# mp3guy/Kintinuous

Hardware: NVIDIA H100
Metric: frames/s 640x480 into 512^3 TSDF (ICP-only tracker) (higher is better)
Workload: dtype f32

## Files before the change

### kintinuous_b200/csrc/kt_capi.cu

```cuda
#include "kt_ops.h"
#include "kt_solve.cuh"
#include "kt_pgo.hpp"
#include "../../include/kintinuous_b200.h"
#include <cstring>
#include <cstddef>
#include <mutex>
#include <vector>
#include <algorithm>

using namespace kt;

namespace {

Intr intr4(const float* k) { Intr r = {k[0], k[1], k[2], k[3]}; return r; }
Mat33 mat33(const float* m) { Mat33 r; r.r0 = make_float3(m[0], m[1], m[2]); r.r1 = make_float3(m[3], m[4], m[5]); r.r2 = make_float3(m[6], m[7], m[8]); return r; }
cudaStream_t st(void* s) { return (cudaStream_t)s; }

struct OpScratch { Allocations mem; OdomState* state; float* partials; int* ipartials; unsigned int* counter; OdomState* host_state;
                   DeviceBuffer<float> ztable; SliceWorkspace slice_ws; MeshWorkspace mesh_ws; DeviceBuffer<unsigned long long> mesh_cells; SurfWorkspace surf_ws; PnpWorkspace pnp_ws;
                   SliceWorkspace fit_ws; DeviceBuffer<int> place_ints; };
enum { KT_MAX_DEVICES = 64 };
OpScratch* g_ops_dev[KT_MAX_DEVICES];
std::mutex g_ops_mu;
OpScratch& ops_scratch()
{
    int dev = 0;
    if (cudaGetDevice(&dev) != cudaSuccess || dev < 0 || dev >= KT_MAX_DEVICES) dev = 0;
    if (!g_ops_dev[dev]) g_ops_dev[dev] = new OpScratch();
    return *g_ops_dev[dev];
}
#define g_ops (ops_scratch())
#define KT_OPS_LOCK() std::lock_guard<std::mutex> _ops_lock(g_ops_mu)

int ensure_scratch()
{
    if (g_ops.host_state) return 0;
    Allocations m; const char* W = "operator scratch";
    OdomState* state; float* partials; int* ipartials; unsigned int* counter; OdomState* host_state;
    int r;
    if ((r = m.device(&state, 1, W)) || (r = m.device(&partials, (size_t)MAX_PARTIALS * 32, W)) || (r = m.device(&ipartials, (size_t)MAX_PARTIALS * 2, W)) ||
        (r = m.device(&counter, 1, W)) || (r = m.pinned(&host_state, 1, W))) return r;
    KT_CUDA(cudaMemset(state, 0, sizeof(OdomState)));
    OpScratch& o = g_ops;
    o.mem = std::move(m); o.state = state; o.partials = partials; o.ipartials = ipartials; o.counter = counter; o.host_state = host_state;
    return 0;
}
int check_vol(const char* who, int vol)
{
    if (vol <= 0 || vol % 8 != 0) { set_error("%s: vol %d is not a positive multiple of 8", who, vol); return KT_ERR_INVALID; }
    return KT_OK;
}

int ensure_ztable(int vol)
{
    const size_t n = vol > 0 ? (size_t)2 * vol : 0;
    return g_ops.ztable.grow(n, n, "operator z table");
}

}

extern "C" {

int kt_op_bilateral(const uint16_t* src, uint16_t* dst, int rows, int cols, void* s)
{ int r = bilateral(src, dst, rows, cols, st(s)); if (r) return r; KT_CUDA(cudaStreamSynchronize(st(s))); return KT_OK; }

int kt_op_pyrdown(const uint16_t* src, uint16_t* dst, int sr, int sc, void* s)
{ int r = pyrdown(src, dst, sr, sc, st(s)); if (r) return r; KT_CUDA(cudaStreamSynchronize(st(s))); return KT_OK; }

int kt_op_create_vmap(const float* k, const uint16_t* depth, float* vmap, int rows, int cols, void* s)
{ int r = create_vmap(intr4(k), depth, vmap, rows, cols, st(s)); if (r) return r; KT_CUDA(cudaStreamSynchronize(st(s))); return KT_OK; }

int kt_op_create_nmap(const float* vmap, float* nmap, int rows, int cols, void* s)
{ int r = create_nmap(vmap, nmap, rows, cols, st(s)); if (r) return r; KT_CUDA(cudaStreamSynchronize(st(s))); return KT_OK; }

int kt_op_create_maps(const float* k, const uint16_t* depth, float* vmap, float* nmap, int rows, int cols, void* s)
{
    MapsLevel L; L.depth = depth; L.vmap = vmap; L.nmap = nmap; L.rows = rows; L.cols = cols; L.k = intr4(k); L.vstale = 0; L.nstale = 0;
    int r = create_maps_pyramid(&L, 1, st(s)); if (r) return r;
    KT_CUDA(cudaStreamSynchronize(st(s))); return KT_OK;
}

int kt_op_frontend(const uint16_t* depth_raw, const uint8_t* rgb, int rows, int cols, const float* k, int angle_color,
                   uint16_t* const* depths4, float* const* vmaps4, float* const* nmaps4, float* depth_scaled, float* cw, float* rgbf,
                   float* const* depth_m4, uint8_t* const* intensity4, int16_t* const* dIdx4, int16_t* const* dIdy4, void* s)
{
    if (!depth_raw || !rgb || !depths4 || !vmaps4 || !nmaps4) { set_error("kt_op_frontend: null argument"); return KT_ERR_INVALID; }
    int r = bilateral_scale(depth_raw, depths4[0], depth_scaled, rows, cols, intr4(k), angle_color != 0, st(s)); if (r) return r;
    FrontendArgs fa;
    fa.depth_f = depths4[0]; fa.depth_raw = depth_raw; fa.rgb = rgb; fa.rows = rows; fa.cols = cols; fa.k = intr4(k);
    fa.depths = depths4; fa.vmaps = vmaps4; fa.nmaps = nmaps4; fa.vstale = 0; fa.nstale = 0;
    fa.cw = cw; fa.rgbf = (float4*)rgbf; fa.angle_color = angle_color != 0; fa.cut_off = 6000;
// ... 8 lines not shown

int kt_op_resize_vmap(const float* in, float* out, int in_rows, int in_cols, void* s)
{ int r = resize_map(in, out, in_rows, in_cols, false, st(s)); if (r) return r; KT_CUDA(cudaStreamSynchronize(st(s))); return KT_OK; }

int kt_op_resize_nmap(const float* in, float* out, int in_rows, int in_cols, void* s)
{ int r = resize_map(in, out, in_rows, in_cols, true, st(s)); if (r) return r; KT_CUDA(cudaStreamSynchronize(st(s))); return KT_OK; }

int kt_op_icp_step(const float* Rcurr, const float* tcurr, const float* vmap_curr, const float* nmap_curr,
                   const float* Rprev_inv, const float* tprev, const float* k,
                   const float* vmap_g_prev, const float* nmap_g_prev, int rows, int cols,
                   float dist_thres, float angle_thres, float* A_host, float* b_host, float* residual_host, void* s)
{
    KT_OPS_LOCK();
    int r = ensure_scratch(); if (r) return r;
    OdomState* h = g_ops.host_state;
    std::memset(h, 0, sizeof(OdomState));
    std::memcpy(h->Rcurr, Rcurr, 36); std::memcpy(h->tcurr, tcurr, 12); std::memcpy(h->Rprev_inv, Rprev_inv, 36); std::memcpy(h->tprev, tprev, 12);
    KT_CUDA(cudaMemcpyAsync(g_ops.state, h, sizeof(OdomState), cudaMemcpyHostToDevice, st(s)));
    IcpLevelArgs a = {vmap_curr, nmap_curr, vmap_g_prev, nmap_g_prev, rows, cols, intr4(k), dist_thres, angle_thres};
    r = icp_iteration(a, g_ops.state, g_ops.partials, 0, 0, st(s)); if (r) return r;
    KT_CUDA(cudaMemcpyAsync(h->sums_icp, (char*)g_ops.state + offsetof(OdomState, sums_icp), 32 * sizeof(float), cudaMemcpyDeviceToHost, st(s)));
    KT_CUDA(cudaStreamSynchronize(st(s)));
    unpack_normal_equations(h->sums_icp, A_host, b_host);
    residual_host[0] = h->sums_icp[27]; residual_host[1] = h->sums_icp[28];
    return KT_OK;
}

int kt_op_integrate(const uint16_t* depth_raw, int rows, int cols, const float* k, const float* vs,
                    const float* Rinv, const float* t, float trunc, int16_t* tsdf, uint8_t* color, int vol,
                    const int* wrap, const uint8_t* rgb, const float* nmap_curr, int angle_color, float* depth_scaled, void* s)
{
    int r = check_vol("kt_op_integrate", vol); if (r) return r;
    KT_OPS_LOCK();
    r = ensure_ztable(vol); if (r) return r;
    r = scale_depth(depth_raw, depth_scaled, rows, cols, intr4(k), angle_color != 0, st(s)); if (r) return r;
    IntegrateArgs a; a.cw = 0; a.rgbf = 0; a.reset_words = 0; a.reset_count = 0; a.reset_stride = 1;
    a.depth_scaled = depth_scaled; a.rows = rows; a.cols = cols; a.k = intr4(k); a.volume_size = make_float3(vs[0], vs[1], vs[2]);
    a.Rinv = mat33(Rinv); a.t = make_float3(t[0], t[1], t[2]); a.trunc = trunc; a.tsdf = tsdf; a.color = color; a.vol = vol;
    a.wrap = make_int3(wrap[0], wrap[1], wrap[2]); a.rgb = rgb; a.nmap_curr = nmap_curr; a.angle_color = angle_color != 0;
    a.multi = 0; a.vv = single_volume(tsdf, color, vol);
    r = integrate(a, g_ops.ztable.get(), st(s)); if (r) return r;
    KT_CUDA(cudaStreamSynchronize(st(s)));
    return KT_OK;
}

int kt_op_raycast(const float* k, const float* R, const float* t, float trunc, const float* vs,
                  const int16_t* tsdf, int vol, float* vmap, float* nmap, int rows, int cols,
                  const int* wrap, uint8_t* vmap_color, const uint8_t* color, void* s)
{
    if (vol > 0) { if (int r = check_cell_size(make_float3(vs[0], vs[1], vs[2]), vol)) return r; }
    if (int r = check_vol("kt_op_raycast", vol)) return r;
    RaycastArgs a = {};
    a.k = intr4(k); a.R = mat33(R); a.t = make_float3(t[0], t[1], t[2]); a.trunc = trunc; a.volume_size = make_float3(vs[0], vs[1], vs[2]);
    a.tsdf = tsdf; a.color = color; a.vol = vol; a.wrap = make_int3(wrap[0], wrap[1], wrap[2]);
    for (int l = 0; l < LEVELS; ++l) { a.vmap[l] = vmap; a.nmap[l] = nmap; }
    a.rows = rows; a.cols = cols; a.vmap_color = vmap_color; a.n_levels = 1;
    int r = raycast(a, st(s)); if (r) return r;
    KT_CUDA(cudaStreamSynchronize(st(s)));
    return KT_OK;
}

int kt_op_extract_slice(const int16_t* tsdf, const float* vs, int vol, kt_point_xyzrgb* out, size_t capacity,
                        const int* wrap, const uint8_t* color, int minX, int maxX, int minY, int maxY, int minZ, int maxZ,
                        int subsample, const int* real_wrap, size_t* count, void* s)
{
    int r = check_vol("kt_op_extract_slice", vol); if (r) return r;
    KT_OPS_LOCK();
    r = ensure_scratch(); if (r) return r;
    KT_CUDA(cudaMemsetAsync(g_ops.counter, 0, sizeof(unsigned int), st(s)));
    r = extract_slice(tsdf, make_float3(vs[0], vs[1], vs[2]), vol, out, capacity, make_int3(wrap[0], wrap[1], wrap[2]), color,
                      minX, maxX, minY, maxY, minZ, maxZ, subsample, make_int3(real_wrap[0], real_wrap[1], real_wrap[2]), g_ops.counter, st(s));
    if (r) return r;
    unsigned int n = 0;
    KT_CUDA(cudaMemcpyAsync(&n, g_ops.counter, sizeof(n), cudaMemcpyDeviceToHost, st(s)));
// ... 296 lines not shown
```

### kintinuous_b200/csrc/kt_ops.h

```cpp
#pragma once
#include "kt_common.cuh"
#include "kt_mem.hpp"
#include <functional>

struct kt_deform_report;
struct kt_pgo_report;
struct kt_weld_report;
struct kt_global_mesh_report;

namespace kt {

static const int LEVELS = 4;
static const int MAX_GPUS = 8;

struct VolumeView {
    int16_t* tsdf[MAX_GPUS];
    uint8_t* color[MAX_GPUS];
    int world, rank, bshift, nshift;
};
__host__ __device__ __forceinline__ int vv_owner(const VolumeView& v, int sz) { return (sz >> v.bshift) & (v.world - 1); }
__host__ __device__ __forceinline__ int vv_local_plane(const VolumeView& v, int sz)
{ return ((sz >> (v.bshift + v.nshift)) << v.bshift) | (sz & ((1 << v.bshift) - 1)); }
inline VolumeView single_volume(int16_t* tsdf, uint8_t* color, int V)
{
// ... 61 lines not shown

int icp_frame(const IcpLevelArgs* levels, const int* iters, const float* pose12_host, OdomState* state, unsigned long long* xwords_dev,
              float* trace, int* timeout_dev, long long* prof_dev, float* host_pose, unsigned int host_seq, cudaStream_t s,
              unsigned long long* const* peer_words = 0, int world = 1, int rank = 0);
size_t odom_exchange_words();
int odom_exchange_used(int* stride);
int odom_exchange_reset(unsigned long long* xwords_dev, cudaStream_t s);

struct RgbLevelArgs {
    const int16_t* dIdx; const int16_t* dIdy; const float* last_depth; const float* next_depth;
    const uint8_t* last_image; const uint8_t* next_image; void* corres; const float* cloud;
    int rows, cols; float min_scale, max_depth_delta, fx, fy, sobel_scale; double Kfx, Kfy, Kcx, Kcy;
};
int rgb_residual(const RgbLevelArgs& a, OdomState* state, int* partials, int use_state_warp, cudaStream_t s);
int rgbd_frame(const IcpLevelArgs* icp_levels, const RgbLevelArgs* rgb_levels, const int* iters, int with_icp, const float* pose12_host, OdomState* state,
               unsigned long long* xwords_dev, float* trace, int* timeout_dev, float* host_pose, unsigned int host_seq, cudaStream_t s);
int rgb_iteration(const RgbLevelArgs& a, OdomState* state, float* partials, float* trace, int mode, float sigma_override, cudaStream_t s);
int odom_begin_frame(OdomState* state, const float* pose12_dev, cudaStream_t s);
int reduce_grid_for(int n_items);

int init_volume(int16_t* tsdf, uint8_t* color, int vol, cudaStream_t s);
int init_shared(const VolumeView& vv, int vol, cudaStream_t s);
int clear_volume(int axis, int back, int16_t* tsdf, uint8_t* color, int vol, int current_wrap, int delta_wrap, cudaStream_t s);
int clear_volume_shared(int axis, int back, const VolumeView& vv, int vol, int current_wrap, int delta_wrap, cudaStream_t s);
void clear_range(int axis, int back, int vol, int current_wrap, int delta_wrap, int* first, int* planes);
int scale_depth(const uint16_t* depth, float* scaled, int rows, int cols, const Intr& k, bool angle_color, cudaStream_t s);
struct IntegrateArgs {
    const float* depth_scaled; int rows, cols; Intr k; float3 volume_size; Mat33 Rinv; float3 t; float trunc;
    int16_t* tsdf; uint8_t* color; int vol; int3 wrap; const uint8_t* rgb; const float* nmap_curr; bool angle_color;
    int multi; VolumeView vv;
    float* cw; float4* rgbf;
    unsigned long long* reset_words; int reset_count, reset_stride;
};
int integrate(const IntegrateArgs& a, float* ztable_dev , cudaStream_t s);
struct RaycastArgs {
    Intr k; Mat33 R; float3 t; float trunc; float3 volume_size; const int16_t* tsdf; const uint8_t* color; int vol; int3 wrap;
    float* vmap[LEVELS]; float* nmap[LEVELS]; int rows, cols; uint8_t* vmap_color; int n_levels;
    int multi; VolumeView vv; int tile_row_begin, tile_row_end;
    float* peer_vmap[MAX_GPUS][LEVELS]; float* peer_nmap[MAX_GPUS][LEVELS]; uint8_t* peer_vcol[MAX_GPUS];
};
int raycast(const RaycastArgs& a, cudaStream_t s);
int check_cell_size(const float3& volume_size, int vol);
int extract_slice(const int16_t* tsdf, const float3& volume_size, int vol, void* out, size_t capacity, const int3& wrap,
                  const uint8_t* color, int minX, int maxX, int minY, int maxY, int minZ, int maxZ, int subsample,
                  const int3& real_wrap, unsigned int* counter_dev, cudaStream_t s);
int extract_slice_mg(const VolumeView& vv, const float3& volume_size, int vol, void* out, size_t capacity, const int3& wrap,
                     int minX, int maxX, int minY, int maxY, int minZ, int maxZ, int subsample,
                     const int3& real_wrap, unsigned int* counter_dev, cudaStream_t s);
struct SliceWorkspace {
    DeviceBuffer<unsigned int> mask, word_off, block_tot;
    DeviceBuffer<unsigned char> acc;
    Allocations fixed; unsigned int* bounds = nullptr; unsigned int* bounds_host = nullptr;
};
int process_slice(const void* points_dev , size_t n, int weight_cull, float leaf, int k_search, void* out_dev ,
                  size_t capacity, size_t* count, SliceWorkspace* ws, cudaStream_t s);
struct MeshArgs {
    const int16_t* tsdf; const uint8_t* color; int vol; float3 volume_size; int3 wrap; int3 real_wrap;
    int minX, maxX, minY, maxY, minZ, maxZ; int weight_cull;
};
struct MeshWorkspace {
    DeviceBuffer<unsigned long long> counts;
    DeviceBuffer<unsigned char> tmp;
    DeviceBuffer<unsigned long long> keys;
    Allocations fixed; unsigned long long* totals_host = nullptr;
};
int mesh_count(const MeshArgs& a, MeshWorkspace* ws, size_t* n_verts, size_t* n_tris, cudaStream_t s);
int mesh_emit(const MeshArgs& a, MeshWorkspace* ws, size_t n_verts, void* verts, uint32_t* tris, cudaStream_t s, unsigned long long* vkeys = nullptr,
// ... 71 lines not shown
```

### kintinuous_b200/csrc/kt_tracker.cu

```cuda
#include "kt_ops.h"
#include "kt_shift.hpp"
#include "kt_posegraph.hpp"
#include "kt_deform.hpp"
#include "kt_pgo.hpp"
#include "kt_place.hpp"
#include <cstdlib>
#include "../../include/kintinuous_b200.h"
#include <memory>
#include <vector>
#include <unordered_map>
#include <cstring>
#include <cmath>
#include <climits>
#include <algorithm>
#include <cstdarg>
#include <cstdio>

namespace kt {

static thread_local char g_err[512] = "";
std::atomic<long long> g_launches(0);
void set_error(const char* fmt, ...)
{
    va_list ap; va_start(ap, fmt); vsnprintf(g_err, sizeof(g_err), fmt, ap); va_end(ap);
// ... 114 lines not shown
    int* best; float* d1; float* d2; unsigned char* pass; int* seg_passes;
    float* pn; float* po; float* uv; double* pose; unsigned char* inl; int* ninl; PnpWorkspace pnp_ws;
    MapPyramid maps[2];
    OdomState* state; unsigned long long* xwords; float* trace;
    kt_point_xyzrgb* cloud[2]; kt_point_xyzrgbnormal* cent[2]; double* d2fit; SliceWorkspace ws[2];
    std::vector<std::vector<float> > in_new, in_old;
    ~PlaceStore() { if (stream) cudaStreamSynchronize(stream); }
};

}

using namespace kt;

struct kt_ctx {
    kt_config cfg;
    cudaStream_t stream;
    float size, voxel, trunc;
    float volumeBasis[3], currentGlobalCamera[3];
    int voxelWrap[3];
    int global_time; uint64_t current_utime;
    int overlap, parked;
    std::vector<M3> rmats; std::vector<V3> tvecs;
    std::vector<SliceRec> slices;
    std::vector<kt_dense_pose> dense_poses;
    FILE* pose_log;
    int iterations[LEVELS];
    int16_t* tsdf; uint8_t* color;
    FrameInputs in, in_spare; FrontEnd fe, fe_spare;
    const void* pf_depth; const void* pf_rgb; bool pf_valid;
    bool pf_built;
    bool frontend_ready;
    cudaStream_t stream_copy; cudaEvent_t ev_prefetch, ev_done[2], ev_maps; int last_parity; bool maps_on_stream;
    float* vmaps_g_prev[LEVELS]; float* nmaps_g_prev[LEVELS];
    uint8_t* vmap_curr_color; float* ztable;
    unsigned long long* xwords_dev; bool xwords_clean;
    OdomState* state; float* partials; int* ipartials; float* trace_dev; float* pose12_dev; long long* prof_dev;
    kt_point_xyzrgb* cloud_dev; unsigned int* counter_dev; size_t cloud_capacity; size_t cloud_count;
    PinnedArena slice_arena; cudaStream_t stream_slices; cudaEvent_t ev_cloud_ready, ev_cloud_free; bool cloud_busy;
    int slice_processing, slice_weight_cull; SliceWorkspace slice_ws; DeviceBuffer<kt_point_xyzrgbnormal> proc; size_t proc_count;
    int slice_meshing, mesh_weight_cull; MeshWorkspace mesh_ws; DeviceBuffer<kt_mesh_vertex> mesh_verts; DeviceBuffer<uint32_t> mesh_tris;
    size_t mesh_nv, mesh_nt;
    DeviceBuffer<unsigned long long> mesh_vkeys, mesh_tcells; MeshKeyFrame mesh_frame;
    struct Deformed { kt_point_xyzrgbnormal* processed; kt_mesh_vertex* mesh_verts; };
    std::vector<Deformed> deformed; PinnedArena deform_arena;
    struct Loop { uint64_t time1, time2; double C[16]; std::vector<float> in1, in2; };
    std::vector<Loop> loops; std::vector<kt_dense_pose> pgo_nodes;
    struct MapCorrection { uint64_t time; float tracked[16]; float corrected[16]; };
    MapCorrection map_corr;
    PhotometricPyramid ph_last, ph_next;
    int16_t* nextdIdx[LEVELS]; int16_t* nextdIdy[LEVELS]; float* pointClouds[LEVELS]; void* corresImg[LEVELS];
    float* pose12_host; OdomResult* result_host; float* result_dev_alias; unsigned int pose_seq; float* trace_host; unsigned int* counter_host;
    int trace_iters; int shifted_last;
    bool timing; cudaEvent_t ev[6]; cudaEvent_t ev_icp[2]; cudaEvent_t ev_krn[4]; cudaEvent_t ev_span[2];
    long long launches_at_create;
    Allocations mem;
    int world, rank, local_planes, mg_block;
    uint8_t* arena; size_t arena_bytes;
    size_t off_tsdf, off_color, off_vmap[LEVELS], off_nmap[LEVELS], off_vcol, off_flags, off_xwords;
    bool split_icp;
    uint8_t* peer_arena[MAX_GPUS]; bool connected;
    unsigned int** peer_flags_dev; unsigned int epoch; int* mg_error_dev; int* mg_error_host;
    VolumeView vv;
    float last_int_Rinv[9], last_int_t[3]; int last_int_wrap[3];
    DeviceBuffer<uint8_t> view;
    std::unique_ptr<PlaceStore> place;
    std::unique_ptr<MapVolume> mapvol;
    bool mapvol_restore = false;
// ... 93 lines not shown
        KT_CUDA(cudaEventRecord(c->ev_cloud_free, c->stream_slices));
        c->cloud_busy = true;
    }
    for (int i = 0; i < 3; ++i) s.camera_t[i] = c->currentGlobalCamera[i];
    for (int i = 0; i < 9; ++i) s.camera_R[i] = c->rmats.back().m[i];
    s.utime = c->current_utime;
    c->slices.push_back(std::move(s));
    return 0;
}

void drop_slices(kt_ctx* c)
{
    if (c->stream_slices) cudaStreamSynchronize(c->stream_slices);
    c->slices.clear();
    c->slice_arena.rewind();
    c->cloud_busy = false;
}

bool builds_icp_maps(const kt_config& cfg) { return cfg.odometry == 0 || cfg.odometry == 2 || cfg.angle_color; }

int do_integrate(kt_ctx* c, const M3& Rinv, const V3& t, const int* wrap)
{
    const int rows = c->cfg.rows, cols = c->cfg.cols;
    Intr k = {c->cfg.fx, c->cfg.fy, c->cfg.cx, c->cfg.cy};
    IntegrateArgs a;
    a.depth_scaled = c->fe.depth_scaled; a.rows = rows; a.cols = cols; a.k = k; a.volume_size = make_float3(c->size, c->size, c->size);
    a.Rinv = to_mat33(Rinv.m); a.t = make_float3(t.v[0], t.v[1], t.v[2]); a.trunc = c->trunc;
    a.tsdf = c->tsdf; a.color = c->color; a.vol = c->cfg.vol; a.wrap = make_int3(wrap[0], wrap[1], wrap[2]);
    a.rgb = c->in.rgb; a.nmap_curr = c->fe.maps.nmaps[0]; a.angle_color = c->cfg.angle_color != 0;
    for (int k = 0; k < 9; ++k) c->last_int_Rinv[k] = Rinv.m[k];
    for (int k = 0; k < 3; ++k) { c->last_int_t[k] = t.v[k]; c->last_int_wrap[k] = wrap[k]; }
    a.reset_words = c->xwords_dev; a.reset_count = odom_exchange_used(&a.reset_stride); c->xwords_clean = true;
    a.multi = c->world > 1 ? 1 : 0; a.vv = c->vv; a.cw = builds_icp_maps(c->cfg) ? c->fe.cw : 0; a.rgbf = a.cw ? (float4*)c->fe.rgbf : 0;
    return integrate(a, c->ztable, c->stream);
}

struct OdomMaps { const float* const* vmaps_curr; const float* const* nmaps_curr; const float* const* vmaps_g_prev; const float* const* nmaps_g_prev; };

void odom_level_args(const kt_ctx* c, const OdomMaps& m, int level, IcpLevelArgs* ia, RgbLevelArgs* ra)
{
    const float distThres = 0.10f, angleThres = sinf(20.f * 3.14159254f / 180.f);
    const Intr K = {c->cfg.fx, c->cfg.fy, c->cfg.cx, c->cfg.cy};
    const int lr = c->cfg.rows >> level, lc = c->cfg.cols >> level;
    const Intr kl = intr_level(K, level);
    const IcpLevelArgs icp = {m.vmaps_curr[level], m.nmaps_curr[level], m.vmaps_g_prev[level], m.nmaps_g_prev[level], lr, lc, kl, distThres, angleThres};
    *ia = icp;
    if (c->cfg.odometry == 0) return;
    const double SOBEL_SCALE = 1.0 / std::pow(2.0, 3);
    const int minimumGradientMagnitudes[4] = {12, 5, 3, 1};
    const int div = 1 << level;
    ra->dIdx = c->nextdIdx[level]; ra->dIdy = c->nextdIdy[level]; ra->last_depth = c->ph_last.depth[level]; ra->next_depth = c->ph_next.depth[level];
    ra->last_image = c->ph_last.image[level]; ra->next_image = c->ph_next.image[level]; ra->corres = c->corresImg[level]; ra->cloud = c->pointClouds[level];
    ra->rows = lr; ra->cols = lc;
    ra->min_scale = (float)(std::pow((double)minimumGradientMagnitudes[level], 2.0) / std::pow(SOBEL_SCALE, 2.0));
    ra->max_depth_delta = 0.07f; ra->fx = kl.fx; ra->fy = kl.fy; ra->sobel_scale = (float)SOBEL_SCALE;
    ra->Kfx = (double)K.fx / div; ra->Kfy = (double)K.fy / div; ra->Kcx = (double)K.cx / div; ra->Kcy = (double)K.cy / div;
}

int run_odometry(kt_ctx* c, const OdomMaps& maps, const M3& Rprev, const V3& tprev, M3* Rcurr, V3* tcurr)
{
    const int mode = c->cfg.odometry;
    int r;
    for (int k = 0; k < 9; ++k) c->pose12_host[k] = Rprev.m[k];
    for (int k = 0; k < 3; ++k) c->pose12_host[9 + k] = tprev.v[k];
    IcpLevelArgs la[LEVELS]; RgbLevelArgs ra[LEVELS];
    for (int level = 0; level < LEVELS; ++level) odom_level_args(c, maps, level, &la[level], &ra[level]);
    int total_iters = 0;
// ... 381 lines not shown
        if (dev(&c->arena, off)) return KT_ERR_CUDA;
        KT_CUDA(cudaMemset(c->arena + c->off_flags, 0, 256));
        c->xwords_dev = (unsigned long long*)(c->arena + c->off_xwords);
        KT_CUDA(cudaMemset(c->xwords_dev, 0, odom_exchange_words() * sizeof(unsigned long long))); c->xwords_clean = true;
        c->split_icp = c->world > 1 && getenv("KT_MG_SPLIT_ICP") != nullptr;
        c->tsdf = (int16_t*)(c->arena + c->off_tsdf); c->color = c->arena + c->off_color;
        for (int g = 0; g < MAX_GPUS; ++g) c->peer_arena[g] = c->arena;
        c->connected = (c->world == 1);
        c->epoch = 0;
        c->vv = single_volume(c->tsdf, c->color, cfg->vol);
        c->vv.world = c->world; c->vv.rank = c->rank;
        c->vv.bshift = 0; { int t = c->mg_block; while (t > 1) { t >>= 1; ++c->vv.bshift; } }
        c->vv.nshift = 0; { int t = c->world; while (t > 1) { t >>= 1; ++c->vv.nshift; } }
        if (dev(&c->peer_flags_dev, (size_t)MAX_GPUS)) return KT_ERR_CUDA;
        if (c->mem.mapped(&c->mg_error_host, 1, W)) return KT_ERR_CUDA; *c->mg_error_host = 0;
        KT_CUDA(cudaHostGetDevicePointer((void**)&c->mg_error_dev, c->mg_error_host, 0));
    }
    if (c->in.alloc(c->mem, P, W) || c->in_spare.alloc(c->mem, P, W) || c->fe.alloc(c->mem, P, W) || c->fe_spare.alloc(c->mem, P, W)) return KT_ERR_CUDA;
    if (cfg->odometry != 0 && (c->ph_last.alloc(c->mem, P, W) || c->ph_next.alloc(c->mem, P, W))) return KT_ERR_CUDA;
    if (c->mem.stream(&c->stream_copy, W)) return KT_ERR_CUDA;
    if (event(&c->ev_prefetch, cudaEventDisableTiming)) return KT_ERR_CUDA;
    for (int i = 0; i < 2; ++i) if (event(&c->ev_done[i], cudaEventDisableTiming)) return KT_ERR_CUDA;
    if (event(&c->ev_maps, cudaEventDisableTiming)) return KT_ERR_CUDA; c->maps_on_stream = false;
    c->last_parity = 0;
    for (int l = 0; l < LEVELS; ++l) {
        size_t Pl = P >> (2 * l);
        c->vmaps_g_prev[l] = (float*)(c->arena + c->off_vmap[l]); c->nmaps_g_prev[l] = (float*)(c->arena + c->off_nmap[l]);
        if (cfg->odometry != 0) {
            if (dev(&c->nextdIdx[l], Pl) || dev(&c->nextdIdy[l], Pl)) return KT_ERR_CUDA;
            if (dev(&c->pointClouds[l], Pl * 3)) return KT_ERR_CUDA;
            uint8_t* ci = 0; if (dev(&ci, Pl * 16)) return KT_ERR_CUDA; c->corresImg[l] = ci;
        }
    }
    c->vmap_curr_color = c->arena + c->off_vcol; if (dev(&c->ztable, (size_t)2 * cfg->vol)) return KT_ERR_CUDA;

    if (dev(&c->state, 1) || dev(&c->partials, (size_t)MAX_PARTIALS * 32)) return KT_ERR_CUDA;
    KT_CUDA(cudaMemset(c->partials, 0, (size_t)MAX_PARTIALS * 32 * sizeof(float)));
    if (dev(&c->prof_dev, 64 * 8) || dev(&c->ipartials, (size_t)MAX_PARTIALS * 2)) return KT_ERR_CUDA;
    if (dev(&c->trace_dev, (size_t)MAX_TRACE_ITERS * TRACE_STRIDE) || dev(&c->pose12_dev, 12)) return KT_ERR_CUDA;
    c->cloud_capacity = (size_t)c->cfg.cloud_capacity;
    if (dev(&c->cloud_dev, c->cloud_capacity) || dev(&c->counter_dev, 1)) return KT_ERR_CUDA;
    c->mesh_weight_cull = 8;
    if (!c->slice_arena.alloc(256)) return KT_ERR_CUDA;
    c->slice_arena.rewind();
    if (c->mem.stream(&c->stream_slices, W)) return KT_ERR_CUDA;
    if (event(&c->ev_cloud_ready, cudaEventDisableTiming)) return KT_ERR_CUDA;
    if (event(&c->ev_cloud_free, cudaEventDisableTiming)) return KT_ERR_CUDA;
    if (c->mem.pinned(&c->pose12_host, 12, W)) return KT_ERR_CUDA;
    if (c->mem.mapped(&c->result_host, 1, W)) return KT_ERR_CUDA;
    std::memset(c->result_host, 0, sizeof(OdomResult));
    { void* dp = 0; KT_CUDA(cudaHostGetDevicePointer(&dp, c->result_host, 0)); c->result_dev_alias = (float*)dp; }
    c->pose_seq = 0;
    if (c->mem.pinned(&c->trace_host, (size_t)MAX_TRACE_ITERS * TRACE_STRIDE, W)) return KT_ERR_CUDA;
    if (c->mem.pinned(&c->counter_host, 1, W)) return KT_ERR_CUDA;
    for (int i = 0; i < 6; ++i) if (event(&c->ev[i], cudaEventDefault)) return KT_ERR_CUDA;
    for (int i = 0; i < 2; ++i) if (event(&c->ev_icp[i], cudaEventDefault)) return KT_ERR_CUDA;
    for (int i = 0; i < 4; ++i) if (event(&c->ev_krn[i], cudaEventDefault)) return KT_ERR_CUDA;
    for (int i = 0; i < 2; ++i) if (event(&c->ev_span[i], cudaEventDefault)) return KT_ERR_CUDA;
    int r = kt_reset(c); if (r) return r;
    *out = owner.release();
    return KT_OK;
}

int kt_destroy(kt_ctx* c)
{
    delete c;
    return KT_OK;
// ... 1364 lines not shown
```

### kintinuous_b200/csrc/kt_tsdf.cu

```cuda
#include "kt_ops.h"
#include "kt_replay.cuh"
#include "kt_frustum.hpp"

namespace kt {

namespace {

__global__ void __launch_bounds__(256) fill_zero_u4(uint4* __restrict__ p, size_t n16)
{
    const uint4 z = make_uint4(0, 0, 0, 0);
    for (size_t i = (size_t)blockIdx.x * blockDim.x + threadIdx.x; i < n16; i += (size_t)gridDim.x * blockDim.x) p[i] = z;
}

__global__ void __launch_bounds__(256)
clear_planes_yz_kernel(int16_t* __restrict__ tsdf, uint8_t* __restrict__ color, int V, int axis, int p0, int count, const VolumeView vv)
{
    const int xg = V / 8;
    const size_t total = (size_t)count * V * xg;
    const uint4 z4 = make_uint4(0, 0, 0, 0);
    for (size_t idx = (size_t)blockIdx.x * blockDim.x + threadIdx.x; idx < total; idx += (size_t)gridDim.x * blockDim.x) {
        int g = (int)(idx % xg);
        size_t r = idx / xg;
        int other = (int)(r % V);
        int i = (int)(r / V);
        int plane = p0 + i; if (plane >= V) plane -= V;
        int sy = axis == 1 ? plane : other;
        int sz = axis == 1 ? other : plane;
        *reinterpret_cast<uint4*>(tsdf + ((size_t)sz * V + sy) * V + (size_t)g * 8) = z4;
        if (vv_owner(vv, sz) != vv.rank) continue;
        size_t base = ((size_t)vv_local_plane(vv, sz) * V + sy) * V + (size_t)g * 8;
        uint4* c = reinterpret_cast<uint4*>(color + base * 4);
        c[0] = z4; c[1] = z4;
    }
}

__global__ void __launch_bounds__(256)
clear_planes_x_kernel(int16_t* __restrict__ tsdf, uchar4* __restrict__ color, int V, int p0, int count, const VolumeView vv)
{
    const size_t total = (size_t)count * V * V;
    for (size_t idx = (size_t)blockIdx.x * blockDim.x + threadIdx.x; idx < total; idx += (size_t)gridDim.x * blockDim.x) {
        int i = (int)(idx % count);
        size_t r = idx / count;
        int sx = p0 + i; if (sx >= V) sx -= V;
        const int sz = (int)(r / V), sy = (int)(r - (size_t)sz * V);
        tsdf[r * V + sx] = 0;
        if (vv_owner(vv, sz) != vv.rank) continue;
        color[((size_t)vv_local_plane(vv, sz) * V + sy) * V + sx] = make_uchar4(0, 0, 0, 0);
    }
}

__global__ void __launch_bounds__(256) ztable_kernel(float* __restrict__ table, int V, float cell_z, float t_z, unsigned long long* __restrict__ reset_words, int reset_count, int reset_stride, int seq)
{
    const int i = blockIdx.x * blockDim.x + threadIdx.x;
    if (blockIdx.x == 0) for (int k = threadIdx.x; k < reset_count; k += blockDim.x) reset_words[(size_t)k * reset_stride] = 0ull;
    if (i >= 2 * V) return;
    const int z = i < V ? i : i - V;
    float v = i < V ? __fmaf_rn(0.5f, cell_z, -t_z) : 0.f;
    if (seq) { for (int k = 0; k < z; ++k) v = __fadd_rn(v, cell_z); }
    else v = replay_add(v, cell_z, z);
    table[i] = v;
}

struct IntegrateParams {
    const float* depth_scaled; int rows, cols; Intr k; float3 cell; Mat33 Rinv; float3 t; float trunc;
    int16_t* tsdf; uchar4* color; int V; int3 wrap; const uint8_t* rgb; const float* nmap; bool angle_color;
    const float* ztable; int zchunk;
    const float* cw; const float4* rgbf;
    int lz_lo, lz_hi;
    int z_far_first;
    VolumeView vv;
    int tile_x0, tiles_x, tile_y0, tiles_y;
    int seq_replay;
};

#define KT_MAX_WEIGHT 128
#define KT_RGB_VIEW_ANGLE_WEIGHT 0.75f

__device__ __forceinline__ unsigned int sat_u8_rn(float x)
{
    unsigned int r;
    asm("cvt.rni.sat.u8.f32 %0, %1;" : "=r"(r) : "f"(x));
    return r;
}

template <typename IdxT, int ZU, int MINB, bool PREP = false, bool MG = false>
__global__ void __launch_bounds__(256, MINB)
integrate_kernel(const IntegrateParams p)
{
    const int V = p.V;
    int bx = p.tile_x0 + (int)blockIdx.x; if (bx >= p.tiles_x) bx -= p.tiles_x;
    int by = p.tile_y0 + (int)blockIdx.y; if (by >= p.tiles_y) by -= p.tiles_y;
    const int sx = bx * 32 + threadIdx.x;
    const int sy = by * 8 + threadIdx.y;
    const int z0 = p.lz_lo + (p.z_far_first ? (int)(gridDim.z - 1 - blockIdx.z) : (int)blockIdx.z) * p.zchunk;
    const int z1 = min(z0 + p.zchunk, p.lz_hi);

    const float3 cell_size = p.cell;
    const Intr intr = p.k;
    const Mat33 Rcurr_inv = p.Rinv;
    const float3 tcurr = p.t;
    const float tranc_dist = p.trunc;
    const int cols = p.cols, rows = p.rows;

    if (sx >= V || sy >= V) return;
    int x = sx - p.wrap.x; if (x < 0) x += V;
    int y = sy - p.wrap.y; if (y < 0) y += V;

    float v_g_x = __fmaf_rn(x + 0.5f, cell_size.x, -tcurr.x);
    float v_g_y = __fmaf_rn(y + 0.5f, cell_size.y, -tcurr.y);
    float v_g_z = __fmaf_rn(0.5f, cell_size.z, -tcurr.z);

    float v_g_part_norm = __fmaf_rn(v_g_x, v_g_x, __fmul_rn(v_g_y, v_g_y));

    float v_x = __fmul_rn(__fmaf_rn(Rcurr_inv.r0.z, v_g_z, __fmaf_rn(Rcurr_inv.r0.x, v_g_x, __fmul_rn(Rcurr_inv.r0.y, v_g_y))), intr.fx);
    float v_y = __fmul_rn(__fmaf_rn(Rcurr_inv.r1.z, v_g_z, __fmaf_rn(Rcurr_inv.r1.x, v_g_x, __fmul_rn(Rcurr_inv.r1.y, v_g_y))), intr.fy);
    float v_z = __fmaf_rn(Rcurr_inv.r2.z, v_g_z, __fmaf_rn(Rcurr_inv.r2.x, v_g_x, __fmul_rn(Rcurr_inv.r2.y, v_g_y)));

    float Rcurr_inv_0_z_scaled = Rcurr_inv.r0.z * cell_size.z * intr.fx;
    float Rcurr_inv_1_z_scaled = Rcurr_inv.r1.z * cell_size.z * intr.fy;
    const float m0z = __fmul_rn(Rcurr_inv.r0.z, cell_size.z), m1z = __fmul_rn(Rcurr_inv.r1.z, cell_size.z);

    float tranc_dist_inv = 1.0f / tranc_dist;

    int zlo = z0, zhi = z1;
    {
        const float dqx = Rcurr_inv_0_z_scaled, dqy = Rcurr_inv_1_z_scaled, dqz = Rcurr_inv.r2.z * cell_size.z;
        {
            const float za = (float)(z0 - 3), zb = (float)(z1 + 3);
// ... 8 lines not shown
        float lo = -1e30f, hi = 1e30f;
        const float ca[5] = { v_z,
                              v_x + (intr.cx + 1.5f) * v_z,
                              -(v_x + (intr.cx - cols - 0.5f) * v_z),
                              v_y + (intr.cy + 1.5f) * v_z,
                              -(v_y + (intr.cy - rows - 0.5f) * v_z) };
        const float cb[5] = { dqz,
                              dqx + (intr.cx + 1.5f) * dqz,
                              -(dqx + (intr.cx - cols - 0.5f) * dqz),
                              dqy + (intr.cy + 1.5f) * dqz,
                              -(dqy + (intr.cy - rows - 0.5f) * dqz) };
#pragma unroll
        for (int c = 0; c < 5; ++c) {
            const float a = ca[c], b = cb[c];
            const float eps = 1e-3f * (fabsf(a) + fabsf(b) * V) + 1e-6f;
            if (fabsf(b) * V <= eps) { if (a < -eps) { lo = 1e30f; hi = -1e30f; } }
            else {
                float zc = -(a + eps) / b;
                if (b > 0) lo = fmaxf(lo, zc); else hi = fminf(hi, zc);
            }
        }
        if (lo > hi) return;
        zlo = max(z0, (int)floorf(fmaxf(lo, -4.f)) - 2);
        zhi = min(z1, (int)ceilf(fminf(hi, (float)V + 4.f)) + 3);
        if (zlo >= zhi) return;
    }

    if (p.seq_replay) {
        for (int z = 0; z < zlo; ++z) { v_x = __fmaf_rn(m0z, intr.fx, v_x); v_y = __fmaf_rn(m1z, intr.fy, v_y); }
    } else {
        v_x = replay_fma(v_x, m0z, intr.fx, zlo);
        v_y = replay_fma(v_y, m1z, intr.fy, zlo);
    }
    const float* __restrict__ zt = p.ztable;
    const float* __restrict__ depthScaled = p.depth_scaled;
    const float* __restrict__ nmap_curr = p.nmap;
    const uchar3* __restrict__ colors = reinterpret_cast<const uchar3*>(p.rgb);
    const IdxT P = (IdxT)rows * cols;
    const IdxT plane = (IdxT)V * V;
    const IdxT col_off = (IdxT)sy * V + sx;

    for (int zb = zlo; zb < zhi; zb += ZU) {
        if (MG) {
            int sz = zb + p.wrap.z; if (sz >= V) sz -= V;
            if (vv_owner(p.vv, sz) != p.vv.rank) {
                const int blk = sz >> p.vv.bshift;
                const int foreign = (p.vv.rank - blk - 1) & (p.vv.world - 1);
                int skip = (((blk + 1) << p.vv.bshift) - sz) + (foreign << p.vv.bshift);
                skip = min(skip, zhi - zb);
                if (skip <= 48) { for (int k = 0; k < skip; ++k) { v_x = __fmaf_rn(m0z, intr.fx, v_x); v_y = __fmaf_rn(m1z, intr.fy, v_y); } }
                else { v_x = replay_fma(v_x, m0z, intr.fx, skip); v_y = replay_fma(v_y, m1z, intr.fy, skip); }
                zb += skip - ZU;
                continue;
            }
        }
        float vgz[ZU], Dp[ZU];
        IdxT pix[ZU], addr[ZU], caddr[ZU];
        bool ok[ZU];
        float nx[ZU], nz[ZU];
        int16_t tprev[ZU]; uchar4 cprev[ZU]; uchar3 rgbv[ZU]; float4 rgbq[ZU];
#pragma unroll
        for (int u = 0; u < ZU; ++u) {
            const int z = zb + u;
            ok[u] = false;
            if (z < zhi) {
                vgz[u] = zt[z];
                const float z_scaled = zt[V + z];
                float inv_z = 1.0f / __fmaf_rn(Rcurr_inv.r2.z, z_scaled, v_z);
                if (!(inv_z < 0)) {
                    int2 coo = { __float2int_rn(__fmaf_rn(v_x, inv_z, intr.cx)), __float2int_rn(__fmaf_rn(v_y, inv_z, intr.cy)) };
                    if (coo.x >= 0 && coo.y >= 0 && coo.x < cols && coo.y < rows) {
                        int sz = z + p.wrap.z; if (sz >= V) sz -= V;
                        ok[u] = true;
                        pix[u] = (IdxT)coo.y * cols + coo.x;
                        addr[u] = (IdxT)sz * plane + col_off;
                        caddr[u] = MG ? (IdxT)vv_local_plane(p.vv, sz) * plane + col_off : addr[u];
                        Dp[u] = depthScaled[pix[u]];
                    }
                }
                v_x = __fmaf_rn(m0z, intr.fx, v_x);
                v_y = __fmaf_rn(m1z, intr.fy, v_y);
            }
        }
        bool upd[ZU], nocol[ZU];
        float tsdf_new[ZU];
#pragma unroll
        for (int u = 0; u < ZU; ++u) {
            upd[u] = false;
            if (ok[u]) {
                float Dp_scaled = Dp[u];
                bool no_color = false;
                if (Dp_scaled < 0.0) { Dp_scaled = -Dp_scaled; no_color = true; }
                float sdf = Dp_scaled - sqrtf(__fmaf_rn(vgz[u], vgz[u], v_g_part_norm));
                if (Dp_scaled != 0 && sdf >= -tranc_dist) {
                    upd[u] = true; nocol[u] = no_color;
                    tsdf_new[u] = fmin(1.0f, sdf * tranc_dist_inv);
                    tprev[u] = p.tsdf[addr[u]];
                    cprev[u] = p.color[caddr[u]];
                    if (PREP) { nx[u] = p.cw[pix[u]]; rgbq[u] = p.rgbf[pix[u]]; }
                    else {
// ... 92 lines not shown
    const int n = delta - current;
    const int an = n < 0 ? -n : n;
    const int base = wrap_base(current, V);
    int p0 = back ? ((base - an) % V + V) % V : base;
    int count = an + 1;
    if (axis == 0) {
        int reach = (an % 16 != 0) ? (an + 16 - an % 16) : an;
        if (count > reach) count = reach;
    }
    if (count > V) count = V;
    *first = p0; *planes = count > 0 ? count : 0;
}

int clear_volume_shared(int axis, int back, const VolumeView& vv, int vol, int current, int delta, cudaStream_t s)
{
    const int V = vol;
    int p0, count;
    clear_range(axis, back, vol, current, delta, &p0, &count);
    if (count <= 0) return 0;
    int16_t* tsdf = vv.tsdf[vv.rank]; uint8_t* color = vv.color[vv.rank];
    if (axis == 0) {
        size_t total = (size_t)count * V * V;
        int grid = (int)((total + 255) / 256 < (size_t)device_info().sm_count * 16 ? (total + 255) / 256 : (size_t)device_info().sm_count * 16);
        clear_planes_x_kernel<<<grid, 256, 0, s>>>(tsdf, (uchar4*)color, V, p0, count, vv);
    } else {
        size_t total = (size_t)count * V * (V / 8);
        int grid = (int)((total + 255) / 256 < (size_t)device_info().sm_count * 16 ? (total + 255) / 256 : (size_t)device_info().sm_count * 16);
        clear_planes_yz_kernel<<<grid, 256, 0, s>>>(tsdf, color, V, axis, p0, count, vv);
    }
    KT_LAUNCH_CHECK();
    return 0;
}

int integrate(const IntegrateArgs& a, float* ztable_dev, cudaStream_t s)
{
    const int V = a.vol;
    float3 cell = make_float3(a.volume_size.x / V, a.volume_size.y / V, a.volume_size.z / V);
    static const bool seq_replay = getenv("KT_INT_SEQ_REPLAY") != nullptr;
    ztable_kernel<<<div_up(2 * V, 256), 256, 0, s>>>(ztable_dev, V, cell.z, a.t.z, a.reset_words, a.reset_words ? a.reset_count : 0, a.reset_stride, seq_replay ? 1 : 0);
    KT_LAUNCH_CHECK();
    IntegrateParams p;
    p.depth_scaled = a.depth_scaled; p.rows = a.rows; p.cols = a.cols; p.k = a.k; p.cell = cell; p.Rinv = a.Rinv; p.t = a.t; p.trunc = a.trunc;
    p.tsdf = a.tsdf; p.color = (uchar4*)a.color; p.V = V; p.wrap = wrap_mod3(a.wrap, V); p.rgb = a.rgb; p.nmap = a.nmap_curr; p.angle_color = a.angle_color;
    static int zu = -1;
    if (zu < 0) { const char* e = getenv("KT_INT_ZU"); zu = e ? atoi(e) : 0; }
    static int prep_knob = -1;
    if (prep_knob < 0) { const char* e = getenv("KT_INT_PREP"); prep_knob = e ? atoi(e) : 1; }
    const bool prep = prep_knob != 0 && a.cw && a.rgbf;
    p.cw = a.cw; p.rgbf = a.rgbf;
    p.ztable = ztable_dev; p.zchunk = V >= 64 ? (V + 15) / 16 : V;
    p.z_far_first = a.Rinv.r2.z > 0.f ? 0 : 1;
    const bool multi = a.multi && a.vv.world > 1;
    p.vv = multi ? a.vv : single_volume(a.tsdf, a.color, V);
    static const bool force64 = getenv("KT_FORCE_IDX64") != nullptr;
    const bool idx32 = !force64 && (size_t)V * V * V <= ((size_t)1 << 31);
    p.lz_lo = 0; p.lz_hi = V;
    p.seq_replay = seq_replay ? 1 : 0;
    p.tiles_x = div_up(V, 32); p.tiles_y = div_up(V, 8); p.tile_x0 = 0; p.tile_y0 = 0;
    dim3 block(32, 8), grid(p.tiles_x, p.tiles_y, div_up(V, p.zchunk));
    static const bool no_box = getenv("KT_INT_NOBOX") != nullptr;
    if (!no_box) {
        const float Rinv9[9] = {a.Rinv.r0.x, a.Rinv.r0.y, a.Rinv.r0.z, a.Rinv.r1.x, a.Rinv.r1.y, a.Rinv.r1.z, a.Rinv.r2.x, a.Rinv.r2.y, a.Rinv.r2.z};
        const float t3[3] = {a.t.x, a.t.y, a.t.z}, k4[4] = {a.k.fx, a.k.fy, a.k.cx, a.k.cy}, cell3[3] = {cell.x, cell.y, cell.z};
        const VoxelBox box = frustum_voxel_box(Rinv9, t3, k4, a.rows, a.cols, V, cell3);
        if (box.empty) return 0;
        p.lz_lo = box.lo[2]; p.lz_hi = box.hi[2] + 1;
        grid.z = div_up(p.lz_hi - p.lz_lo, p.zchunk);
        if (V % 32 == 0) { int n; cyclic_tile_range(box.lo[0], box.hi[0], p.wrap.x, V, 32, &p.tile_x0, &n); grid.x = n; }
        if (V % 8 == 0) { int n; cyclic_tile_range(box.lo[1], box.hi[1], p.wrap.y, V, 8, &p.tile_y0, &n); grid.y = n; }
    }
    if (multi) {
        if (V & (V - 1)) { set_error("integrate: the shared volume needs a power-of-two resolution"); return -1; }
        if (idx32) { if (prep) integrate_kernel<unsigned int, 1, 6, true, true><<<grid, block, 0, s>>>(p); else integrate_kernel<unsigned int, 1, 6, false, true><<<grid, block, 0, s>>>(p); }
        else { if (prep) integrate_kernel<size_t, 1, 6, true, true><<<grid, block, 0, s>>>(p); else integrate_kernel<size_t, 1, 6, false, true><<<grid, block, 0, s>>>(p); }
    } else if (idx32) {
        const int variant = zu ? zu : (V >= 1024 ? 1 : 2);
        if (prep && (variant == 1 || variant == 2)) {
            if (variant == 1) integrate_kernel<unsigned int, 1, 6, true><<<grid, block, 0, s>>>(p);
            else integrate_kernel<unsigned int, 2, 4, true><<<grid, block, 0, s>>>(p);
        } else
        if (variant == 1) integrate_kernel<unsigned int, 1, 6><<<grid, block, 0, s>>>(p);
        else integrate_kernel<unsigned int, 2, 4><<<grid, block, 0, s>>>(p);
    }
    else if (prep) integrate_kernel<size_t, 1, 6, true><<<grid, block, 0, s>>>(p);
    else integrate_kernel<size_t, 1, 6><<<grid, block, 0, s>>>(p);
    KT_LAUNCH_CHECK();
    return 0;
}

namespace {
__global__ void xgpu_barrier_kernel(unsigned int* const* peer_flags, volatile unsigned int* my_flags, int rank, int world, unsigned int epoch, int* error)
{
    const int t = threadIdx.x;
    if (t < world) {
        __threadfence_system();
        volatile unsigned int* dst = peer_flags[t] + rank;
        *dst = epoch;
        __threadfence_system();
        const long long t0 = clock64();
        while ((int)(my_flags[t] - epoch) < 0) {
            if (clock64() - t0 > 4000000000LL) { *error = 1 + t; break; }
        }
        __threadfence_system();
    }
}
}

int xgpu_barrier(unsigned int* const* peer_flags_dev, unsigned int* my_flags, int rank, int world, unsigned int epoch, int* error_dev, cudaStream_t s)
{
    xgpu_barrier_kernel<<<1, 32, 0, s>>>(peer_flags_dev, my_flags, rank, world, epoch, error_dev);
    KT_LAUNCH_CHECK();
    return 0;
}

}
```

Measured before the change: 3314.

## Fold z-table kernel into integrate via host chunk seeds and shared memory

Removes the separate ztable kernel launch and its global buffer. The host now computes per-chunk starting values with sequential FTZ float adds, and each integrate block rebuilds its slice of the z table in shared memory. The block at grid index (0,0,0) now clears the exchange reset words, with a small fallback kernel for the empty-frustum case. This saves one launch per frame and the global table reads, but adds a serial shared-memory fill by one thread per block plus a sync, and it drops the seq_replay/replay_add path for the table.

```diff
diff --git a/kintinuous_b200/csrc/kt_capi.cu b/kintinuous_b200/csrc/kt_capi.cu
--- a/kintinuous_b200/csrc/kt_capi.cu
+++ b/kintinuous_b200/csrc/kt_capi.cu
@@ -17,7 +17,7 @@
 cudaStream_t st(void* s) { return (cudaStream_t)s; }
 
 struct OpScratch { Allocations mem; OdomState* state; float* partials; int* ipartials; unsigned int* counter; OdomState* host_state;
-                   DeviceBuffer<float> ztable; SliceWorkspace slice_ws; MeshWorkspace mesh_ws; DeviceBuffer<unsigned long long> mesh_cells; SurfWorkspace surf_ws; PnpWorkspace pnp_ws;
+                   SliceWorkspace slice_ws; MeshWorkspace mesh_ws; DeviceBuffer<unsigned long long> mesh_cells; SurfWorkspace surf_ws; PnpWorkspace pnp_ws;
                    SliceWorkspace fit_ws; DeviceBuffer<int> place_ints; };
 enum { KT_MAX_DEVICES = 64 };
 OpScratch* g_ops_dev[KT_MAX_DEVICES];
@@ -51,12 +51,6 @@
     return KT_OK;
 }
 
-int ensure_ztable(int vol)
-{
-    const size_t n = vol > 0 ? (size_t)2 * vol : 0;
-    return g_ops.ztable.grow(n, n, "operator z table");
-}
-
 }
 
 extern "C" {
@@ -131,14 +125,13 @@
 {
     int r = check_vol("kt_op_integrate", vol); if (r) return r;
     KT_OPS_LOCK();
-    r = ensure_ztable(vol); if (r) return r;
     r = scale_depth(depth_raw, depth_scaled, rows, cols, intr4(k), angle_color != 0, st(s)); if (r) return r;
     IntegrateArgs a; a.cw = 0; a.rgbf = 0; a.reset_words = 0; a.reset_count = 0; a.reset_stride = 1;
     a.depth_scaled = depth_scaled; a.rows = rows; a.cols = cols; a.k = intr4(k); a.volume_size = make_float3(vs[0], vs[1], vs[2]);
     a.Rinv = mat33(Rinv); a.t = make_float3(t[0], t[1], t[2]); a.trunc = trunc; a.tsdf = tsdf; a.color = color; a.vol = vol;
     a.wrap = make_int3(wrap[0], wrap[1], wrap[2]); a.rgb = rgb; a.nmap_curr = nmap_curr; a.angle_color = angle_color != 0;
     a.multi = 0; a.vv = single_volume(tsdf, color, vol);
-    r = integrate(a, g_ops.ztable.get(), st(s)); if (r) return r;
+    r = integrate(a, st(s)); if (r) return r;
     KT_CUDA(cudaStreamSynchronize(st(s)));
     return KT_OK;
 }
diff --git a/kintinuous_b200/csrc/kt_ops.h b/kintinuous_b200/csrc/kt_ops.h
--- a/kintinuous_b200/csrc/kt_ops.h
+++ b/kintinuous_b200/csrc/kt_ops.h
@@ -117,7 +117,7 @@
     float* cw; float4* rgbf;
     unsigned long long* reset_words; int reset_count, reset_stride;
 };
-int integrate(const IntegrateArgs& a, float* ztable_dev , cudaStream_t s);
+int integrate(const IntegrateArgs& a, cudaStream_t s);
 struct RaycastArgs {
     Intr k; Mat33 R; float3 t; float trunc; float3 volume_size; const int16_t* tsdf; const uint8_t* color; int vol; int3 wrap;
     float* vmap[LEVELS]; float* nmap[LEVELS]; int rows, cols; uint8_t* vmap_color; int n_levels;
diff --git a/kintinuous_b200/csrc/kt_tracker.cu b/kintinuous_b200/csrc/kt_tracker.cu
--- a/kintinuous_b200/csrc/kt_tracker.cu
+++ b/kintinuous_b200/csrc/kt_tracker.cu
@@ -170,7 +170,7 @@
     bool frontend_ready;
     cudaStream_t stream_copy; cudaEvent_t ev_prefetch, ev_done[2], ev_maps; int last_parity; bool maps_on_stream;
     float* vmaps_g_prev[LEVELS]; float* nmaps_g_prev[LEVELS];
-    uint8_t* vmap_curr_color; float* ztable;
+    uint8_t* vmap_curr_color;
     unsigned long long* xwords_dev; bool xwords_clean;
     OdomState* state; float* partials; int* ipartials; float* trace_dev; float* pose12_dev; long long* prof_dev;
     kt_point_xyzrgb* cloud_dev; unsigned int* counter_dev; size_t cloud_capacity; size_t cloud_count;
@@ -330,7 +330,7 @@
     for (int k = 0; k < 3; ++k) { c->last_int_t[k] = t.v[k]; c->last_int_wrap[k] = wrap[k]; }
     a.reset_words = c->xwords_dev; a.reset_count = odom_exchange_used(&a.reset_stride); c->xwords_clean = true;
     a.multi = c->world > 1 ? 1 : 0; a.vv = c->vv; a.cw = builds_icp_maps(c->cfg) ? c->fe.cw : 0; a.rgbf = a.cw ? (float4*)c->fe.rgbf : 0;
-    return integrate(a, c->ztable, c->stream);
+    return integrate(a, c->stream);
 }
 
 struct OdomMaps { const float* const* vmaps_curr; const float* const* nmaps_curr; const float* const* vmaps_g_prev; const float* const* nmaps_g_prev; };
@@ -778,7 +778,7 @@
             uint8_t* ci = 0; if (dev(&ci, Pl * 16)) return KT_ERR_CUDA; c->corresImg[l] = ci;
         }
     }
-    c->vmap_curr_color = c->arena + c->off_vcol; if (dev(&c->ztable, (size_t)2 * cfg->vol)) return KT_ERR_CUDA;
+    c->vmap_curr_color = c->arena + c->off_vcol;
 
     if (dev(&c->state, 1) || dev(&c->partials, (size_t)MAX_PARTIALS * 32)) return KT_ERR_CUDA;
     KT_CUDA(cudaMemset(c->partials, 0, (size_t)MAX_PARTIALS * 32 * sizeof(float)));
diff --git a/kintinuous_b200/csrc/kt_tsdf.cu b/kintinuous_b200/csrc/kt_tsdf.cu
--- a/kintinuous_b200/csrc/kt_tsdf.cu
+++ b/kintinuous_b200/csrc/kt_tsdf.cu
@@ -1,3 +1,5 @@
+#include <cfloat>
+#include <cmath>
 #include "kt_ops.h"
 #include "kt_replay.cuh"
 #include "kt_frustum.hpp"
@@ -49,22 +51,19 @@
     }
 }
 
-__global__ void __launch_bounds__(256) ztable_kernel(float* __restrict__ table, int V, float cell_z, float t_z, unsigned long long* __restrict__ reset_words, int reset_count, int reset_stride, int seq)
-{
-    const int i = blockIdx.x * blockDim.x + threadIdx.x;
-    if (blockIdx.x == 0) for (int k = threadIdx.x; k < reset_count; k += blockDim.x) reset_words[(size_t)k * reset_stride] = 0ull;
-    if (i >= 2 * V) return;
-    const int z = i < V ? i : i - V;
-    float v = i < V ? __fmaf_rn(0.5f, cell_z, -t_z) : 0.f;
-    if (seq) { for (int k = 0; k < z; ++k) v = __fadd_rn(v, cell_z); }
-    else v = replay_add(v, cell_z, z);
-    table[i] = v;
-}
+__global__ void __launch_bounds__(64) reset_words_kernel(unsigned long long* __restrict__ words, int count, int stride)
+{
+    for (int k = threadIdx.x; k < count; k += blockDim.x) words[(size_t)k * stride] = 0ull;
+}
+
+#define KT_MAX_ZCHUNKS 16
 
 struct IntegrateParams {
     const float* depth_scaled; int rows, cols; Intr k; float3 cell; Mat33 Rinv; float3 t; float trunc;
     int16_t* tsdf; uchar4* color; int V; int3 wrap; const uint8_t* rgb; const float* nmap; bool angle_color;
-    const float* ztable; int zchunk;
+    int zchunk;
+    float vgz0[KT_MAX_ZCHUNKS], zs0[KT_MAX_ZCHUNKS];
+    unsigned long long* reset_words; int reset_count, reset_stride;
     const float* cw; const float4* rgbf;
     int lz_lo, lz_hi;
     int z_far_first;
@@ -92,8 +91,19 @@
     int by = p.tile_y0 + (int)blockIdx.y; if (by >= p.tiles_y) by -= p.tiles_y;
     const int sx = bx * 32 + threadIdx.x;
     const int sy = by * 8 + threadIdx.y;
-    const int z0 = p.lz_lo + (p.z_far_first ? (int)(gridDim.z - 1 - blockIdx.z) : (int)blockIdx.z) * p.zchunk;
+    const int chunk = p.z_far_first ? (int)(gridDim.z - 1 - blockIdx.z) : (int)blockIdx.z;
+    const int z0 = p.lz_lo + chunk * p.zchunk;
     const int z1 = min(z0 + p.zchunk, p.lz_hi);
+
+    extern __shared__ float zt_s[];
+    if (threadIdx.x == 0 && threadIdx.y < 2) {
+        float v = threadIdx.y == 0 ? p.vgz0[chunk] : p.zs0[chunk];
+        float* dst = zt_s + threadIdx.y * p.zchunk;
+        for (int i = 0; i < z1 - z0; ++i) { dst[i] = v; v = __fadd_rn(v, p.cell.z); }
+    }
+    if (blockIdx.x == 0 && blockIdx.y == 0 && blockIdx.z == 0)
+        for (int k = threadIdx.y * 32 + threadIdx.x; k < p.reset_count; k += 256) p.reset_words[(size_t)k * p.reset_stride] = 0ull;
+    __syncthreads();
 
     const float3 cell_size = p.cell;
     const Intr intr = p.k;
@@ -168,7 +178,7 @@
         v_x = replay_fma(v_x, m0z, intr.fx, zlo);
         v_y = replay_fma(v_y, m1z, intr.fy, zlo);
     }
-    const float* __restrict__ zt = p.ztable;
+    const float* zt = zt_s - z0;
     const float* __restrict__ depthScaled = p.depth_scaled;
     const float* __restrict__ nmap_curr = p.nmap;
     const uchar3* __restrict__ colors = reinterpret_cast<const uchar3*>(p.rgb);
@@ -201,7 +211,7 @@
             ok[u] = false;
             if (z < zhi) {
                 vgz[u] = zt[z];
-                const float z_scaled = zt[V + z];
+                const float z_scaled = zt[p.zchunk + z];
                 float inv_z = 1.0f / __fmaf_rn(Rcurr_inv.r2.z, z_scaled, v_z);
                 if (!(inv_z < 0)) {
                     int2 coo = { __float2int_rn(__fmaf_rn(v_x, inv_z, intr.cx)), __float2int_rn(__fmaf_rn(v_y, inv_z, intr.cy)) };
@@ -360,14 +370,20 @@
     return 0;
 }
 
-int integrate(const IntegrateArgs& a, float* ztable_dev, cudaStream_t s)
+static float add_ftz(float x, float a)
+{
+    auto ftz = [](float v) { return std::fabs(v) < FLT_MIN ? std::copysign(0.0f, v) : v; };
+    volatile float r = ftz(x) + ftz(a);
+    return ftz(r);
+}
+
+int integrate(const IntegrateArgs& a, cudaStream_t s)
 {
     const int V = a.vol;
     float3 cell = make_float3(a.volume_size.x / V, a.volume_size.y / V, a.volume_size.z / V);
     static const bool seq_replay = getenv("KT_INT_SEQ_REPLAY") != nullptr;
-    ztable_kernel<<<div_up(2 * V, 256), 256, 0, s>>>(ztable_dev, V, cell.z, a.t.z, a.reset_words, a.reset_words ? a.reset_count : 0, a.reset_stride, seq_replay ? 1 : 0);
-    KT_LAUNCH_CHECK();
     IntegrateParams p;
+    p.reset_words = a.reset_words; p.reset_count = a.reset_words ? a.reset_count : 0; p.reset_stride = a.reset_stride;
     p.depth_scaled = a.depth_scaled; p.rows = a.rows; p.cols = a.cols; p.k = a.k; p.cell = cell; p.Rinv = a.Rinv; p.t = a.t; p.trunc = a.trunc;
     p.tsdf = a.tsdf; p.color = (uchar4*)a.color; p.V = V; p.wrap = wrap_mod3(a.wrap, V); p.rgb = a.rgb; p.nmap = a.nmap_curr; p.angle_color = a.angle_color;
     static int zu = -1;
@@ -376,7 +392,7 @@
     if (prep_knob < 0) { const char* e = getenv("KT_INT_PREP"); prep_knob = e ? atoi(e) : 1; }
     const bool prep = prep_knob != 0 && a.cw && a.rgbf;
     p.cw = a.cw; p.rgbf = a.rgbf;
-    p.ztable = ztable_dev; p.zchunk = V >= 64 ? (V + 15) / 16 : V;
+    p.zchunk = V >= 64 ? (V + 15) / 16 : V;
     p.z_far_first = a.Rinv.r2.z > 0.f ? 0 : 1;
     const bool multi = a.multi && a.vv.world > 1;
     p.vv = multi ? a.vv : single_volume(a.tsdf, a.color, V);
@@ -391,27 +407,38 @@
         const float Rinv9[9] = {a.Rinv.r0.x, a.Rinv.r0.y, a.Rinv.r0.z, a.Rinv.r1.x, a.Rinv.r1.y, a.Rinv.r1.z, a.Rinv.r2.x, a.Rinv.r2.y, a.Rinv.r2.z};
         const float t3[3] = {a.t.x, a.t.y, a.t.z}, k4[4] = {a.k.fx, a.k.fy, a.k.cx, a.k.cy}, cell3[3] = {cell.x, cell.y, cell.z};
         const VoxelBox box = frustum_voxel_box(Rinv9, t3, k4, a.rows, a.cols, V, cell3);
-        if (box.empty) return 0;
+        if (box.empty) {
+            if (p.reset_count) { reset_words_kernel<<<1, 64, 0, s>>>(p.reset_words, p.reset_count, p.reset_stride); KT_LAUNCH_CHECK(); }
+            return 0;
+        }
         p.lz_lo = box.lo[2]; p.lz_hi = box.hi[2] + 1;
         grid.z = div_up(p.lz_hi - p.lz_lo, p.zchunk);
         if (V % 32 == 0) { int n; cyclic_tile_range(box.lo[0], box.hi[0], p.wrap.x, V, 32, &p.tile_x0, &n); grid.x = n; }
         if (V % 8 == 0) { int n; cyclic_tile_range(box.lo[1], box.hi[1], p.wrap.y, V, 8, &p.tile_y0, &n); grid.y = n; }
     }
+    {
+        float vgz = add_ftz(0.5f * cell.z, -a.t.z), zs = 0.f;
+        for (int z = 0, k = 0; k < (int)grid.z; ++z) {
+            if (z == p.lz_lo + k * p.zchunk) { p.vgz0[k] = vgz; p.zs0[k] = zs; ++k; }
+            vgz = add_ftz(vgz, cell.z); zs = add_ftz(zs, cell.z);
+        }
+    }
+    const size_t smem = (size_t)2 * p.zchunk * sizeof(float);
     if (multi) {
         if (V & (V - 1)) { set_error("integrate: the shared volume needs a power-of-two resolution"); return -1; }
-        if (idx32) { if (prep) integrate_kernel<unsigned int, 1, 6, true, true><<<grid, block, 0, s>>>(p); else integrate_kernel<unsigned int, 1, 6, false, true><<<grid, block, 0, s>>>(p); }
-        else { if (prep) integrate_kernel<size_t, 1, 6, true, true><<<grid, block, 0, s>>>(p); else integrate_kernel<size_t, 1, 6, false, true><<<grid, block, 0, s>>>(p); }
+        if (idx32) { if (prep) integrate_kernel<unsigned int, 1, 6, true, true><<<grid, block, smem, s>>>(p); else integrate_kernel<unsigned int, 1, 6, false, true><<<grid, block, smem, s>>>(p); }
+        else { if (prep) integrate_kernel<size_t, 1, 6, true, true><<<grid, block, smem, s>>>(p); else integrate_kernel<size_t, 1, 6, false, true><<<grid, block, smem, s>>>(p); }
     } else if (idx32) {
         const int variant = zu ? zu : (V >= 1024 ? 1 : 2);
         if (prep && (variant == 1 || variant == 2)) {
-            if (variant == 1) integrate_kernel<unsigned int, 1, 6, true><<<grid, block, 0, s>>>(p);
-            else integrate_kernel<unsigned int, 2, 4, true><<<grid, block, 0, s>>>(p);
+            if (variant == 1) integrate_kernel<unsigned int, 1, 6, true><<<grid, block, smem, s>>>(p);
+            else integrate_kernel<unsigned int, 2, 4, true><<<grid, block, smem, s>>>(p);
         } else
-        if (variant == 1) integrate_kernel<unsigned int, 1, 6><<<grid, block, 0, s>>>(p);
-        else integrate_kernel<unsigned int, 2, 4><<<grid, block, 0, s>>>(p);
-    }
-    else if (prep) integrate_kernel<size_t, 1, 6, true><<<grid, block, 0, s>>>(p);
-    else integrate_kernel<size_t, 1, 6><<<grid, block, 0, s>>>(p);
+        if (variant == 1) integrate_kernel<unsigned int, 1, 6><<<grid, block, smem, s>>>(p);
+        else integrate_kernel<unsigned int, 2, 4><<<grid, block, smem, s>>>(p);
+    }
+    else if (prep) integrate_kernel<size_t, 1, 6, true><<<grid, block, smem, s>>>(p);
+    else integrate_kernel<size_t, 1, 6><<<grid, block, smem, s>>>(p);
     KT_LAUNCH_CHECK();
     return 0;
 }
```

Result: no change. 3379 (median of 6 runs) (+2.0%).
